# interaction-lab-uh/STROTSS-tensorflow

Measured on AMD Instinct MI355X. Metric: optimisation_steps_per_sec_1024px_pair, higher is better.
Workload: dtype f32; 1 GPU; 1024px content/style pair, 1024x1024 scale of the coarse-to-fine pyramid, 1024 samples x D=2179, VGG16 (seeded He-normal weights), RMSprop pixel update; scale_px=1024, samples=1024, parallelism=single GPU, tap_adjoint=deterministic (planned, sorted scatter)

## Files before the change

strotss-tensorflow_amd/csrc/image.hip:

```cpp
#include "internal.h"

namespace {

struct AxisTap { int lo, hi; float lerp; };
__device__ __forceinline__ AxisTap axis_tap(int i, float scale, int in_size) {
  const float src = __fsub_rn(__fmul_rn(__fadd_rn((float)i, 0.5f), scale), 0.5f);
  const float fl = floorf(src);
  AxisTap t;
  t.lo = max((int)fl, 0);
  t.hi = min((int)ceilf(src), in_size - 1);
  t.lerp = __fsub_rn(src, fl);
  return t;
}

template <int C>
__global__ __launch_bounds__(256) void resize_bilinear_kernel(const float* __restrict__ in, int ih, int iw,
                                                              int c_rt, float* __restrict__ out, int oh, int ow,
                                                              float sy, float sx, float alpha,
                                                              const float* __restrict__ add) {
  const int c = C ? C : c_rt;
  for (int oy = blockIdx.y; oy < oh; oy += gridDim.y) {
    const AxisTap ty = axis_tap(oy, sy, ih);
    const float* r0 = in + (size_t)ty.lo * iw * c;
    const float* r1 = in + (size_t)ty.hi * iw * c;
    const size_t orow = (size_t)oy * ow * c;
    for (int ox = blockIdx.x * 256 + threadIdx.x; ox < ow; ox += gridDim.x * 256) {
      const AxisTap tx = axis_tap(ox, sx, iw);
      const int a = tx.lo * c, b = tx.hi * c;
      const size_t o = orow + (size_t)ox * c;
#pragma unroll
      for (int ch = 0; ch < (C ? C : 1); ++ch)
        for (int cc = ch; cc < c; cc += (C ? C : 1)) {
          const float tl = r0[a + cc], tr = r0[b + cc], bl = r1[a + cc], br = r1[b + cc];
          const float top = tl + (tr - tl) * tx.lerp;
          const float bot = bl + (br - bl) * tx.lerp;
          float v = alpha * (top + (bot - top) * ty.lerp);
          if (add) v += add[o + cc];
          out[o + cc] = v;
        }
    }
  }
}

#define FOLD_TILE 32
#define FOLD_REGION 24
struct FoldLevels { int n; int h[STROTSS_MAX_TENSORS], w[STROTSS_MAX_TENSORS]; const float* v[STROTSS_MAX_TENSORS]; };
__device__ __forceinline__ float bilerp3(float tl, float tr, float bl, float br, float lx, float ly) {
  const float top = tl + (tr - tl) * lx;
  const float bot = bl + (br - bl) * lx;
  return 1.0f * (top + (bot - top) * ly);
}
__global__ __launch_bounds__(256) void fold_pyramid_kernel(FoldLevels p, float* __restrict__ img) {
  __shared__ float buf[2][FOLD_REGION * FOLD_REGION * 3];
  __shared__ int reg[STROTSS_MAX_TENSORS][4];
  const int t = threadIdx.x;
  if (t == 0) {
    int y0 = blockIdx.y * FOLD_TILE, y1 = min(y0 + FOLD_TILE, p.h[0]) - 1;
    int x0 = blockIdx.x * FOLD_TILE, x1 = min(x0 + FOLD_TILE, p.w[0]) - 1;
    reg[0][0] = y0; reg[0][1] = y1; reg[0][2] = x0; reg[0][3] = x1;
    for (int k = 1; k < p.n; ++k) {
      const float sy = (float)p.h[k] / (float)p.h[k - 1], sx = (float)p.w[k] / (float)p.w[k - 1];
      const int ny0 = axis_tap(y0, sy, p.h[k]).lo, ny1 = axis_tap(y1, sy, p.h[k]).hi;
      const int nx0 = axis_tap(x0, sx, p.w[k]).lo, nx1 = axis_tap(x1, sx, p.w[k]).hi;
      y0 = ny0; y1 = ny1; x0 = nx0; x1 = nx1;
      reg[k][0] = y0; reg[k][1] = y1; reg[k][2] = x0; reg[k][3] = x1;
    }
  }
  __syncthreads();
  {
    const int k = p.n - 1, y0 = reg[k][0], x0 = reg[k][2], rh = reg[k][1] - y0 + 1, rw = reg[k][3] - x0 + 1;
    float* dst = buf[k & 1];
    for (int e = t; e < rh * rw; e += 256) {
      const int ry = e / rw, rx = e - ry * rw;
      const float* s = p.v[k] + ((size_t)(y0 + ry) * p.w[k] + x0 + rx) * 3;
      dst[e * 3 + 0] = s[0]; dst[e * 3 + 1] = s[1]; dst[e * 3 + 2] = s[2];
    }
  }
  __syncthreads();
  for (int k = p.n - 2; k >= 0; --k) {
    const int y0 = reg[k][0], x0 = reg[k][2], rh = reg[k][1] - y0 + 1, rw = reg[k][3] - x0 + 1;
    const int cy0 = reg[k + 1][0], cx0 = reg[k + 1][2], cw = reg[k + 1][3] - cx0 + 1;
    const int ih = p.h[k + 1], iw = p.w[k + 1];
    const float sy = (float)ih / (float)p.h[k], sx = (float)iw / (float)p.w[k];
    const float* src = buf[(k + 1) & 1];
    float* dst = k == 0 ? nullptr : buf[k & 1];
    for (int e = t; e < rh * rw; e += 256) {
      const int ry = e / rw, rx = e - ry * rw;
      const int oy = y0 + ry, ox = x0 + rx;
      const AxisTap ty = axis_tap(oy, sy, ih), tx = axis_tap(ox, sx, iw);
      const float* r0 = src + (size_t)(ty.lo - cy0) * cw * 3;
      const float* r1 = src + (size_t)(ty.hi - cy0) * cw * 3;
      const int a = (tx.lo - cx0) * 3, b = (tx.hi - cx0) * 3;
      const size_t o = ((size_t)oy * p.w[k] + ox) * 3;
      const float* add = p.v[k] + o;
#pragma unroll
      for (int c = 0; c < 3; ++c) {
        float v = bilerp3(r0[a + c], r0[b + c], r1[a + c], r1[b + c], tx.lerp, ty.lerp);
        v += add[c];
        if (k == 0) img[o + c] = v; else dst[e * 3 + c] = v;
      }
    }
    __syncthreads();
  }
}

#define ADJ_MAX 8
__device__ __forceinline__ float adj_weight(int o, float scale, int in_size, int i) {
  const AxisTap t = axis_tap(o, scale, in_size);
  return (t.lo == i ? 1.0f - t.lerp : 0.f) + (t.hi == i ? t.lerp : 0.f);
}
struct AdjGlobal3 {
  const float* p; int ow;
  __device__ __forceinline__ const float* at(int oy, int ox) const { return p + ((size_t)oy * ow + ox) * 3; }
};
struct AdjRegion3 {
  const float* p; int y0, x0, rw;
  __device__ __forceinline__ const float* at(int oy, int ox) const { return p + ((oy - y0) * rw + (ox - x0)) * 3; }
};
__device__ __forceinline__ void adj_range(int i, float inv_scale, int out_size, int& o0, int& o1) {
  o0 = max(0, (int)floorf(((float)i - 0.5f) * inv_scale - 0.5f) - 1);
  o1 = min(out_size - 1, (int)ceilf(((float)i + 1.5f) * inv_scale - 0.5f) + 1);
}
template <class Src>
__device__ __forceinline__ void adjoint_pixel3(const Src& g, int oh, int ow, int ih, int iw, float sy, float sx, int iy,
                                               int ix, float (&acc)[3]) {
  int oy0, oy1, ox0, ox1;
  adj_range(iy, 1.0f / sy, oh, oy0, oy1);
  adj_range(ix, 1.0f / sx, ow, ox0, ox1);
  acc[0] = acc[1] = acc[2] = 0.f;
  if (ox1 - ox0 < ADJ_MAX) {
    float wx[ADJ_MAX];
#pragma unroll
    for (int q = 0; q < ADJ_MAX; ++q) wx[q] = (ox0 + q <= ox1) ? adj_weight(ox0 + q, sx, iw, ix) : 0.f;
    for (int oy = oy0; oy <= oy1; ++oy) {
      const float wy = adj_weight(oy, sy, ih, iy);
      if (wy == 0.f) continue;
      float row[3] = {0.f, 0.f, 0.f};
#pragma unroll
      for (int q = 0; q < ADJ_MAX; ++q)
        if (wx[q] != 0.f) {
          const float* p = g.at(oy, ox0 + q);
#pragma unroll
          for (int ch = 0; ch < 3; ++ch) row[ch] += wx[q] * p[ch];
        }
#pragma unroll
      for (int ch = 0; ch < 3; ++ch) acc[ch] += wy * row[ch];
    }
    return;
  }
  for (int oy = oy0; oy <= oy1; ++oy) {
    const float wy = adj_weight(oy, sy, ih, iy);
    if (wy == 0.f) continue;
    float row[3] = {0.f, 0.f, 0.f};
    for (int ox = ox0; ox <= ox1; ++ox) {
      const float w = adj_weight(ox, sx, iw, ix);
      if (w != 0.f) {
        const float* q = g.at(oy, ox);
#pragma unroll
        for (int ch = 0; ch < 3; ++ch) row[ch] += w * q[ch];
      }
    }
#pragma unroll
    for (int ch = 0; ch < 3; ++ch) acc[ch] += wy * row[ch];
  }
}

#define ADJ2_T2 8
#define ADJ2_REGION 32
__global__ __launch_bounds__(256) void resize_adjoint_pair_kernel(const float* __restrict__ g0, int h0, int w0,
                                                                  float* __restrict__ g1, int h1, int w1,
                                                                  float* __restrict__ g2, int h2, int w2) {
  __shared__ float mid[ADJ2_REGION * ADJ2_REGION * 3];
  const int t = threadIdx.x;
  const float sy1 = (float)h1 / (float)h0, sx1 = (float)w1 / (float)w0;
  const float sy2 = (float)h2 / (float)h1, sx2 = (float)w2 / (float)w1;
  const int ty0 = blockIdx.y * ADJ2_T2, ty1 = min(ty0 + ADJ2_T2, h2) - 1, tx0 = blockIdx.x * ADJ2_T2, tx1 = min(tx0 + ADJ2_T2, w2) - 1;
  const int oy0 = blockIdx.y * 2 * ADJ2_T2, oy1 = min(oy0 + 2 * ADJ2_T2, h1) - 1;
  const int ox0 = blockIdx.x * 2 * ADJ2_T2, ox1 = min(ox0 + 2 * ADJ2_T2, w1) - 1;
  const bool has2 = ty0 <= ty1 && tx0 <= tx1, own1 = oy0 <= oy1 && ox0 <= ox1;
  int ry0 = oy0, ry1 = oy1, rx0 = ox0, rx1 = ox1;
  if (has2) {
    int a, b, c, d;
    adj_range(ty0, 1.0f / sy2, h1, a, b); adj_range(ty1, 1.0f / sy2, h1, c, d);
    const int ny0 = a, ny1 = d;
    adj_range(tx0, 1.0f / sx2, w1, a, b); adj_range(tx1, 1.0f / sx2, w1, c, d);
    const int nx0 = a, nx1 = d;
    if (own1) { ry0 = min(ry0, ny0); ry1 = max(ry1, ny1); rx0 = min(rx0, nx0); rx1 = max(rx1, nx1); }
    else { ry0 = ny0; ry1 = ny1; rx0 = nx0; rx1 = nx1; }
  } else if (!own1) {
    return;
  }
  const int rh = ry1 - ry0 + 1, rw = rx1 - rx0 + 1;
  const AdjGlobal3 src0{g0, w0};
  for (int e = t; e < rh * rw; e += 256) {
    const int ry = e / rw, rx = e - ry * rw;
    const int iy = ry0 + ry, ix = rx0 + rx;
    float acc[3];
    adjoint_pixel3(src0, h0, w0, h1, w1, sy1, sx1, iy, ix, acc);
    mid[e * 3 + 0] = acc[0]; mid[e * 3 + 1] = acc[1]; mid[e * 3 + 2] = acc[2];
    if (own1 && iy >= oy0 && iy <= oy1 && ix >= ox0 && ix <= ox1) {
      float* o = g1 + ((size_t)iy * w1 + ix) * 3;
      o[0] = acc[0]; o[1] = acc[1]; o[2] = acc[2];
    }
  }
  __syncthreads();
  if (!has2) return;
  const AdjRegion3 src1{mid, ry0, rx0, rw};
  const int th = ty1 - ty0 + 1, tw = tx1 - tx0 + 1;
  for (int e = t; e < th * tw; e += 256) {
    const int iy = ty0 + e / tw, ix = tx0 + e % tw;
    float acc[3];
    adjoint_pixel3(src1, h1, w1, h2, w2, sy2, sx2, iy, ix, acc);
    float* o = g2 + ((size_t)iy * w2 + ix) * 3;
    o[0] = acc[0]; o[1] = acc[1]; o[2] = acc[2];
  }
}

template <int C>
__global__ __launch_bounds__(256) void resize_adjoint_kernel(const float* __restrict__ gout, int oh, int ow,
                                                             int c_rt, float* __restrict__ gin, int ih, int iw,
                                                             float sy, float sx) {
  const int c = C ? C : c_rt;
  const float isy = 1.0f / sy, isx = 1.0f / sx;
  for (int iy = blockIdx.y; iy < ih; iy += gridDim.y) {
    const int oy0 = max(0, (int)floorf(((float)iy - 0.5f) * isy - 0.5f) - 1);
    const int oy1 = min(oh - 1, (int)ceilf(((float)iy + 1.5f) * isy - 0.5f) + 1);
    for (int ix = blockIdx.x * 256 + threadIdx.x; ix < iw; ix += gridDim.x * 256) {
      const int ox0 = max(0, (int)floorf(((float)ix - 0.5f) * isx - 0.5f) - 1);
      const int ox1 = min(ow - 1, (int)ceilf(((float)ix + 1.5f) * isx - 0.5f) + 1);
      float acc[C ? C : 4];
#pragma unroll
      for (int ch = 0; ch < (C ? C : 4); ++ch) acc[ch] = 0.f;
      if (C && ox1 - ox0 < ADJ_MAX) {
        float wx[ADJ_MAX];
#pragma unroll
        for (int q = 0; q < ADJ_MAX; ++q) wx[q] = (ox0 + q <= ox1) ? adj_weight(ox0 + q, sx, iw, ix) : 0.f;
        for (int oy = oy0; oy <= oy1; ++oy) {
          const float wy = adj_weight(oy, sy, ih, iy);
          if (wy == 0.f) continue;
          const float* g = gout + ((size_t)oy * ow + ox0) * c;
          float row[C ? C : 1];
#pragma unroll
          for (int ch = 0; ch < C; ++ch) row[ch] = 0.f;
#pragma unroll
          for (int q = 0; q < ADJ_MAX; ++q)
            if (wx[q] != 0.f) {
#pragma unroll
              for (int ch = 0; ch < C; ++ch) row[ch] += wx[q] * g[q * c + ch];
            }
#pragma unroll
          for (int ch = 0; ch < C; ++ch) acc[ch] += wy * row[ch];
        }
#pragma unroll
        for (int ch = 0; ch < C; ++ch) gin[((size_t)iy * iw + ix) * c + ch] = acc[ch];
      } else {
        for (int ch0 = 0; ch0 < c; ch0 += 4) {
          const int nc = min(4, c - ch0);
          float a4[4] = {0.f, 0.f, 0.f, 0.f};
          for (int oy = oy0; oy <= oy1; ++oy) {
            const float wy = adj_weight(oy, sy, ih, iy);
            if (wy == 0.f) continue;
            float row[4] = {0.f, 0.f, 0.f, 0.f};
            for (int ox = ox0; ox <= ox1; ++ox) {
              const float w = adj_weight(ox, sx, iw, ix);
              if (w != 0.f)
                for (int ch = 0; ch < nc; ++ch) row[ch] += w * gout[((size_t)oy * ow + ox) * c + ch0 + ch];
            }
            for (int ch = 0; ch < nc; ++ch) a4[ch] += wy * row[ch];
          }
          for (int ch = 0; ch < nc; ++ch) gin[((size_t)iy * iw + ix) * c + ch0 + ch] = a4[ch];
        }
      }
    }
  }
}

struct SampleTap { int ia, ib, ic, id; float wa, wb, wc, wd; };

__device__ __forceinline__ SampleTap sample_tap(const strotss_maps_t& m, int k, float gx, float gy,
                                                int bilinear) {
  for (int q = 0; q < m.n_div[k]; ++q) {
    gx = __fdiv_rn(gx, m.div[q]);
    gy = __fdiv_rn(gy, m.div[q]);
  }
  const int h = m.h[k], w = m.w[k];
  SampleTap t;
  if (bilinear) {
    const float gxf = floorf(gx), gyf = floorf(gy);
    const float dx = gx - gxf, dy = gy - gyf;
    t.wa = (1.f - dx) * (1.f - dy);
    t.wb = (1.f - dx) * dy;
    t.wc = dx * (1.f - dy);
    t.wd = dx * dy;
    const int x0 = (int)fminf(fmaxf(gxf, 0.f), (float)(h - 1));
    const int y0 = (int)fminf(fmaxf(gyf, 0.f), (float)(w - 1));
    int x1 = min(x0 + 1, h - 1);
    const int y1 = min(y0 + 1, w - 1);
    int xa = x0;
    if (m.rows[k] > 0) {
      const int ra = x0 - m.row0[k], rb = x1 - m.row0[k];
      xa = min(max(ra, 0), m.rows[k] - 1);
      x1 = min(max(rb, 0), m.rows[k] - 1);
      if (m.window_drop & (int)(ra != xa)) { t.wa = 0.f; t.wb = 0.f; }
      if (m.window_drop & (int)(rb != x1)) { t.wc = 0.f; t.wd = 0.f; }
    }
    t.ia = xa * w + y0; t.ib = xa * w + y1; t.ic = x1 * w + y0; t.id = x1 * w + y1;
  } else {
    int xi = (int)fminf(fmaxf(gx, 0.f), (float)(h - 1));
    const int yi = (int)fminf(fmaxf(gy, 0.f), (float)(w - 1));
    if (m.rows[k] > 0) xi = min(max(xi - m.row0[k], 0), m.rows[k] - 1);
    t.ia = t.ib = t.ic = t.id = xi * w + yi;
    t.wa = 1.f; t.wb = t.wc = t.wd = 0.f;
  }
  return t;
}

__device__ __forceinline__ void gather_row(const strotss_maps_t& m, const float* __restrict__ idx, int s, int bilinear,
                                           float* __restrict__ out, int ld, int dtotal) {
  if (m.sample_range && (s < m.sample_range[0] || s >= m.sample_range[1])) return;
  const float gx = idx[2 * s], gy = idx[2 * s + 1];
  float* o = out + (size_t)s * ld;
  const int wave = __builtin_amdgcn_readfirstlane((int)threadIdx.x >> 6), lane = threadIdx.x & 63;
  int off = 0, chunk = 0;
  for (int k = 0; k < m.n_maps; ++k) {
    const int c = m.c[k], nchunk = (c + 63) >> 6;
    int q0 = (wave - chunk) & 3;
    if (q0 < nchunk) {
      const SampleTap t = sample_tap(m, k, gx, gy, bilinear);
      const float* src = m.map[k];
      if (bilinear) {
        const float* pa = src + (size_t)t.ia * c; const float* pb = src + (size_t)t.ib * c;
        const float* pc = src + (size_t)t.ic * c; const float* pd = src + (size_t)t.id * c;
        for (int q = q0; q < nchunk; q += 4) {
          const int ch = q * 64 + lane;
          if (ch < c) o[off + ch] = pa[ch] * t.wa + pb[ch] * t.wb + pc[ch] * t.wc + pd[ch] * t.wd;
        }
      } else {
        const float* pa = src + (size_t)t.ia * c;
        for (int q = q0; q < nchunk; q += 4) {
          const int ch = q * 64 + lane;
          if (ch < c) o[off + ch] = pa[ch];
        }
      }
    }
    off += c;
    chunk += nchunk;
  }
  for (int ch = dtotal + threadIdx.x; ch < ld; ch += 256) o[ch] = 0.f;
}
__global__ __launch_bounds__(256) void hypercol_gather_kernel(strotss_maps_t m, const float* __restrict__ idx,
                                                              int bilinear, float* __restrict__ out, int ld,
                                                              int dtotal) {
  gather_row(m, idx, blockIdx.x, bilinear, out, ld, dtotal);
}
__device__ __forceinline__ void gather2_body(const strotss_maps_t& ma, const strotss_maps_t& mb,
                                             const float* __restrict__ idx, int n, int bilinear, float* __restrict__ out_a,
                                             float* __restrict__ out_b, int ld, int dtotal_a, int dtotal_b,
                                             float* __restrict__ zero, int zero_rows, const int b) {
  if (b < n) {
    gather_row(ma, idx, b, bilinear, out_a, ld, dtotal_a);
    if (zero) {
      const int r1 = b == n - 1 ? zero_rows : min(b + 1, zero_rows);
      for (int r = b; r < r1; ++r)
        for (int ch = threadIdx.x; ch < ld; ch += 256) zero[(size_t)r * ld + ch] = 0.f;
    }
  } else {
    gather_row(mb, idx, b - n, bilinear, out_b, ld, dtotal_b);
  }
}
__global__ __launch_bounds__(256) void hypercol_gather2_kernel(strotss_maps_t ma, strotss_maps_t mb,
                                                               const float* __restrict__ idx, int n, int bilinear,
                                                               float* __restrict__ out_a, float* __restrict__ out_b, int ld,
                                                               int dtotal_a, int dtotal_b, float* __restrict__ zero,
                                                               int zero_rows) {
  gather2_body(ma, mb, idx, n, bilinear, out_a, out_b, ld, dtotal_a, dtotal_b, zero, zero_rows, (int)blockIdx.x);
}
__global__ __launch_bounds__(256) void hypercol_gather2_cw_kernel(strotss_maps_t ma, strotss_maps_t mb, strotss_maps_t mw,
                                                                  const float* __restrict__ idx, int n, int bilinear,
                                                                  float* __restrict__ out_a, float* __restrict__ out_b, int ld,
                                                                  int dtotal_a, int dtotal_b, float* __restrict__ zero,
                                                                  int zero_rows, float* __restrict__ wout, int wrows) {
  const int b = blockIdx.x;
  gather2_body(ma, mb, idx, n, bilinear, out_a, out_b, ld, dtotal_a, dtotal_b, zero, zero_rows, b);
  if (b < n) {
    gather_row(mw, idx, b, bilinear, wout, 1, 1);
    if (b == n - 1)
      for (int r = n + (int)threadIdx.x; r < wrows; r += 256) wout[r] = 0.f;
  }
}
#define SCATTER_DENSE_MAX_PIX 64
__device__ __forceinline__ void scatter_dense_block(const strotss_maps_t& m, const float* __restrict__ idx, int n,
                                                    const float* __restrict__ gfeat, int ld, bool masked, int k, int off, int b) {
  __shared__ int li[1024];
  __shared__ float lw[1024];
  __shared__ int cnts[4];
  __shared__ float red[4][64];
  const int tid = threadIdx.x, lane = tid & 63, wave = tid >> 6;
  const int c = m.c[k], nchunk = (c + 63) >> 6;
  const int p = b / nchunk, q = b - p * nchunk;
  const int s0 = m.sample_range ? m.sample_range[0] : 0, s1 = m.sample_range ? min(n, m.sample_range[1]) : n;
  const int ch = q * 64 + lane;
  const bool in = ch < c;
  const float* g = gfeat + off + (in ? ch : c - 1);
  float acc = 0.f;
  for (int base = s0; base < s1; base += 1024) {
    float w4[4];
    int cnt = 0;
#pragma unroll
    for (int u = 0; u < 4; ++u) {
      const int s = base + 4 * tid + u;
      float w = 0.f;
      if (s < s1) {
        const SampleTap t = sample_tap(m, k, idx[2 * s], idx[2 * s + 1], 1);
        w = (t.ia == p ? t.wa : 0.f) + (t.ib == p ? t.wb : 0.f) + (t.ic == p ? t.wc : 0.f) + (t.id == p ? t.wd : 0.f);
      }
      w4[u] = w;
      cnt += w != 0.f;
    }
    int incl = cnt;
#pragma unroll
    for (int o = 1; o < 64; o <<= 1) {
      const int up = __shfl_up(incl, o, 64);
      if (lane >= o) incl += up;
    }
    __syncthreads();
    if (lane == 63) cnts[wave] = incl;
    __syncthreads();
    int at = incl - cnt, total = 0;
#pragma unroll
    for (int wv = 0; wv < 4; ++wv) {
      at += wv < wave ? cnts[wv] : 0;
      total += cnts[wv];
    }
#pragma unroll
    for (int u = 0; u < 4; ++u)
      if (w4[u] != 0.f) { li[at] = base + 4 * tid + u; lw[at] = w4[u]; ++at; }
    __syncthreads();
    int e = wave;
    for (; e + 12 < total; e += 16) {
      float v[4];
#pragma unroll
      for (int u = 0; u < 4; ++u) v[u] = g[(size_t)li[e + 4 * u] * ld];
#pragma unroll
      for (int u = 0; u < 4; ++u) acc += lw[e + 4 * u] * v[u];
    }
    for (; e < total; e += 4) acc += lw[e] * g[(size_t)li[e] * ld];
  }
  red[wave][lane] = acc;
  __syncthreads();
  if (wave == 0 && in) {
    const float tot = (red[0][lane] + red[1][lane]) + (red[2][lane] + red[3][lane]);
    const size_t o = (size_t)p * c + ch;
    if (tot != 0.f && (!masked || m.map[k][o] > 0.f)) m.gmap[k][o] += tot;
  }
}
__global__ __launch_bounds__(256) void hypercol_scatter_kernel(strotss_maps_t m, const float* __restrict__ idx,
                                                               const float* __restrict__ gfeat, int ld,
                                                               int relu_mask_from, int map_begin,
                                                               int map_end, int n, unsigned dense_mask, int dense_blocks) {
  if ((int)blockIdx.x < dense_blocks) {
    int b = (int)blockIdx.x, off = 0;
    for (int k = 0; k < map_end; ++k) {
      if ((dense_mask >> k) & 1u) {
        const int nb = (m.rows[k] > 0 ? m.rows[k] : m.h[k]) * m.w[k] * ((m.c[k] + 63) >> 6);
        if (b < nb) { scatter_dense_block(m, idx, n, gfeat, ld, k >= relu_mask_from, k, off, b); return; }
        b -= nb;
      }
      off += m.c[k];
    }
    return;
  }
  const int s = (int)blockIdx.x - dense_blocks;
  if (m.sample_range && (s < m.sample_range[0] || s >= m.sample_range[1])) return;
  const float gx = idx[2 * s], gy = idx[2 * s + 1];
  const float* g = gfeat + (size_t)s * ld;
  const int wave = __builtin_amdgcn_readfirstlane((int)threadIdx.x >> 6), lane = threadIdx.x & 63;
  int off = 0, chunk = 0;
  for (int k = 0; k < map_end; ++k) {
    const int c = m.c[k], nchunk = (c + 63) >> 6;
    const int q0 = (wave - chunk) & 3;
    chunk += nchunk;
    if (k < map_begin || q0 >= nchunk || ((dense_mask >> k) & 1u)) { off += c; continue; }
    const SampleTap t = sample_tap(m, k, gx, gy, 1);
    const float* act = m.map[k];
    float* dst = m.gmap[k];
    const bool masked = k >= relu_mask_from;
    const int ii[4] = {t.ia, t.ib, t.ic, t.id};
    const float ww[4] = {t.wa, t.wb, t.wc, t.wd};
    for (int q = q0; q < nchunk; q += 4) {
      const int ch = q * 64 + lane;
      const bool in = ch < c;
      const int chc = in ? ch : c - 1;
      const float gv = in ? g[off + chc] : 0.f;
#pragma unroll
      for (int tq = 0; tq < 4; ++tq) {
        const float v = ww[tq] * gv;
        const size_t o = (size_t)ii[tq] * c + chc;
        if (v != 0.f && (!masked || act[o] > 0.f)) atomicAdd(&dst[o], v);
      }
    }
    off += c;
  }
}

#define PLAN_E 4096
struct PlanView {
  int* nseg; int* seg_start; int* pix; int* smp; float* w;
  __host__ __device__ static size_t ints_per_map() { return 2 + (PLAN_E + 1) + 3 * (size_t)PLAN_E + 1; }
  __host__ __device__ PlanView(void* base, int k) {
    int* b = reinterpret_cast<int*>(base) + (size_t)k * ints_per_map();
    nseg = b; seg_start = b + 2; pix = seg_start + PLAN_E + 1; smp = pix + PLAN_E; w = reinterpret_cast<float*>(smp + PLAN_E);
  }
};
__global__ __launch_bounds__(1024) void scatter_plan_kernel(strotss_maps_t m, const float* __restrict__ idx, int n,
                                                            void* __restrict__ plan) {
  __shared__ unsigned long long key[PLAN_E];
  __shared__ int wsum[16];
  const int k = blockIdx.x, t = threadIdx.x;
  const unsigned long long INVALID = ~0ull;
  const int s_begin = m.sample_range ? m.sample_range[0] : 0, s_end = m.sample_range ? min(n, m.sample_range[1]) : n;
  for (int e = t; e < PLAN_E; e += 1024) {
    const int s = e >> 2, q = e & 3;
    unsigned long long kk = INVALID;
    if (s >= s_begin && s < s_end) {
      const SampleTap tp = sample_tap(m, k, idx[2 * s], idx[2 * s + 1], 1);
      const int ii = q == 0 ? tp.ia : q == 1 ? tp.ib : q == 2 ? tp.ic : tp.id;
      const float ww = q == 0 ? tp.wa : q == 1 ? tp.wb : q == 2 ? tp.wc : tp.wd;
      if (ww != 0.f) kk = ((unsigned long long)(unsigned)ii << 12) | (unsigned)e;
    }
    key[e] = kk;
  }
  __syncthreads();
  for (int size = 2; size <= PLAN_E; size <<= 1)
    for (int stride = size >> 1; stride > 0; stride >>= 1) {
      for (int p = t; p < PLAN_E / 2; p += 1024) {
        const int lo = 2 * p - (p & (stride - 1));
        const int hi = lo + stride;
        const bool up = (lo & size) == 0;
        const unsigned long long a = key[lo], b = key[hi];
        if ((a > b) == up) { key[lo] = b; key[hi] = a; }
      }
      __syncthreads();
    }
  PlanView pv(plan, k);
  int head[4], cnt = 0, valid = 0;
#pragma unroll
  for (int i = 0; i < 4; ++i) {
    const int p = 4 * t + i;
    const unsigned long long a = key[p];
    const bool ok = a != INVALID;
    head[i] = ok && (p == 0 || (key[p - 1] >> 12) != (a >> 12));
    cnt += head[i]; valid += ok;
  }
  int incl = cnt, vincl = valid;
#pragma unroll
  for (int o = 1; o < 64; o <<= 1) {
    const int u = __shfl_up(incl, o, 64), v = __shfl_up(vincl, o, 64);
    if ((t & 63) >= o) { incl += u; vincl += v; }
  }
  if ((t & 63) == 63) { wsum[t >> 6] = incl; }
  __syncthreads();
  int base = incl - cnt;
  for (int wv = 0; wv < (t >> 6); ++wv) base += wsum[wv];
  int total = 0;
#pragma unroll
  for (int wv = 0; wv < 16; ++wv) total += wsum[wv];
  __syncthreads();
  if ((t & 63) == 63) wsum[t >> 6] = vincl;
  __syncthreads();
  int nvalid = 0;
#pragma unroll
  for (int wv = 0; wv < 16; ++wv) nvalid += wsum[wv];
#pragma unroll
  for (int i = 0; i < 4; ++i) {
    const int p = 4 * t + i;
    const unsigned long long a = key[p];
    if (a == INVALID) continue;
    const int e = (int)(a & 4095u), s = e >> 2, q = e & 3;
    const SampleTap tp = sample_tap(m, k, idx[2 * s], idx[2 * s + 1], 1);
    pv.pix[p] = (int)(a >> 12);
    pv.smp[p] = s;
    pv.w[p] = q == 0 ? tp.wa : q == 1 ? tp.wb : q == 2 ? tp.wc : tp.wd;
    if (head[i]) pv.seg_start[base++] = p;
  }
  if (t == 0) { pv.nseg[0] = total; pv.seg_start[total] = nvalid; }
}
__global__ __launch_bounds__(256) void scatter_sorted_kernel(strotss_maps_t m, int k, int off, const void* __restrict__ plan,
                                                             const float* __restrict__ gfeat, int ld, int masked) {
  PlanView pv(const_cast<void*>(plan), k);
  const int sg = blockIdx.x;
  if (sg >= pv.nseg[0]) return;
  const int p0 = pv.seg_start[sg], p1 = pv.seg_start[sg + 1];
  const int c = m.c[k];
  const size_t pixel = (size_t)pv.pix[p0] * c;
  const float* act = m.map[k];
  float* dst = m.gmap[k];
  for (int ch = threadIdx.x; ch < c; ch += 256) {
    if (masked && !(act[pixel + ch] > 0.f)) continue;
    float acc = 0.f;
    for (int p = p0; p < p1; ++p) acc += pv.w[p] * gfeat[(size_t)pv.smp[p] * ld + off + ch];
    dst[pixel + ch] += acc;
  }
}

__global__ __launch_bounds__(256) void rmsprop_kernel(strotss_tensors_t t, float lr, float rho, float eps) {
  const int k = blockIdx.y;
  float* var = t.var[k];
  float* rms = t.rms[k];
  const float* g = t.grad[k];
  const int64_t n = t.numel[k];
  const float omr = 1.0f - rho;
  for (int64_t e = (int64_t)blockIdx.x * 256 + threadIdx.x; e < n; e += (int64_t)gridDim.x * 256) {
    const float gv = g[e];
    const float r = rho * rms[e] + omr * (gv * gv);
    rms[e] = r;
    var[e] = var[e] - lr * gv / (sqrtf(r) + eps);
  }
}

__global__ __launch_bounds__(256) void minmax_partial_kernel(const float* __restrict__ x, int64_t n,
                                                             float* __restrict__ ws) {
  __shared__ float red[4];
  float mn = INFINITY, mx = -INFINITY;
  for (int64_t e = (int64_t)blockIdx.x * 256 + threadIdx.x; e < n; e += (int64_t)gridDim.x * 256) {
    const float v = fminf(fmaxf(x[e], 0.f), 1.f);
    mn = fminf(mn, v);
    mx = fmaxf(mx, v);
  }
  mn = block_min_256(mn, red);
  mx = block_max_256(mx, red);
  if (threadIdx.x == 0) { ws[blockIdx.x] = mn; ws[1024 + blockIdx.x] = mx; }
}
__global__ __launch_bounds__(256) void postprocess_kernel(const float* __restrict__ x, int64_t n,
                                                          const float* __restrict__ ws, int nparts,
                                                          uint8_t* __restrict__ out) {
  __shared__ float red[4];
  float mn = INFINITY, mx = -INFINITY;
  for (int i = threadIdx.x; i < nparts; i += 256) { mn = fminf(mn, ws[i]); mx = fmaxf(mx, ws[1024 + i]); }
  mn = block_min_256(mn, red);
  mx = block_max_256(mx, red);
  const float range = mx - mn;
  for (int64_t e = (int64_t)blockIdx.x * 256 + threadIdx.x; e < n; e += (int64_t)gridDim.x * 256) {
    float v = fminf(fmaxf(x[e], 0.f), 1.f);
    v = (v - mn) / range;
    out[e] = (uint8_t)(v * 255.0f);
  }
}

int maps_ok(const strotss_maps_t* m) {
  if (!m || m->n_maps <= 0 || m->n_maps > STROTSS_MAX_MAPS) return 0;
  for (int k = 0; k < m->n_maps; ++k) {
    if (m->h[k] <= 0 || m->w[k] <= 0 || m->c[k] <= 0 || !m->map[k]) return 0;
    if (m->n_div[k] < 0 || m->n_div[k] > STROTSS_MAX_DIVS) return 0;
    if (m->rows[k] < 0 || m->row0[k] < 0 || m->row0[k] + m->rows[k] > m->h[k]) return 0;
  }
  return 1;
}

}

extern "C" {

int strotss_abi_version(void) { return 8; }
const char* strotss_build_info(void) { return "libstrotss_hip gfx950 fp32-mfma " __DATE__ " " __TIME__; }

int strotss_resize_bilinear(const float* in, int ih, int iw, int c, float* out, int oh, int ow, float alpha,
                            const float* add, void* stream) {
  ST_CHECK_ARG(in && out && ih > 0 && iw > 0 && oh > 0 && ow > 0 && c > 0, STROTSS_EINVAL);
  const float sy = (float)ih / (float)oh, sx = (float)iw / (float)ow;
  const dim3 grid((unsigned)cdiv(ow, 256), (unsigned)min(oh, 32768));
  if (c == 3)
    hipLaunchKernelGGL(resize_bilinear_kernel<3>, grid, dim3(256), 0, (hipStream_t)stream, in, ih, iw, c, out, oh, ow, sy, sx,
                       alpha, add);
  else if (c == 1)
    hipLaunchKernelGGL(resize_bilinear_kernel<1>, grid, dim3(256), 0, (hipStream_t)stream, in, ih, iw, c, out, oh, ow, sy, sx,
                       alpha, add);
  else
    hipLaunchKernelGGL(resize_bilinear_kernel<0>, grid, dim3(256), 0, (hipStream_t)stream, in, ih, iw, c, out, oh, ow, sy, sx,
                       alpha, add);
  ST_LAUNCH_RET();
}

int strotss_fold_pyramid(const strotss_pyramid_t* pyr, float* img, void* stream) {
  ST_CHECK_ARG(pyr && img && pyr->n_levels >= 2 && pyr->n_levels <= STROTSS_MAX_TENSORS, STROTSS_EINVAL);
  FoldLevels p;
  p.n = pyr->n_levels;
  for (int k = 0; k < p.n; ++k) {
    ST_CHECK_ARG(pyr->var[k] && pyr->h[k] > 0 && pyr->w[k] > 0, STROTSS_EINVAL);
    p.h[k] = pyr->h[k]; p.w[k] = pyr->w[k]; p.v[k] = pyr->var[k];
  }
  int sy = FOLD_TILE, sx = FOLD_TILE;
  for (int k = 1; k < p.n; ++k) {
    ST_CHECK_ARG(p.h[k] <= p.h[k - 1] && p.w[k] <= p.w[k - 1], STROTSS_ERANGE);
    sy = min(p.h[k], (int)((long long)sy * p.h[k] / p.h[k - 1]) + 3);
    sx = min(p.w[k], (int)((long long)sx * p.w[k] / p.w[k - 1]) + 3);
    ST_CHECK_ARG(sy <= FOLD_REGION && sx <= FOLD_REGION, STROTSS_ERANGE);
  }
  hipLaunchKernelGGL(fold_pyramid_kernel, dim3((unsigned)cdiv(p.w[0], FOLD_TILE), (unsigned)cdiv(p.h[0], FOLD_TILE)), dim3(256),
                     0, (hipStream_t)stream, p, img);
  ST_LAUNCH_RET();
}

static bool adjoint_pair_ok(int a, int b) { return b >= 1 && a >= 2 * b - 1 && a <= 2 * b + 1; }

int strotss_fold_pyramid_adjoint(const strotss_pyramid_t* g, void* stream) {
  ST_CHECK_ARG(g && g->n_levels >= 2 && g->n_levels <= STROTSS_MAX_TENSORS, STROTSS_EINVAL);
  for (int k = 0; k < g->n_levels; ++k) ST_CHECK_ARG(g->var[k] && g->h[k] > 0 && g->w[k] > 0, STROTSS_EINVAL);
  int k = 0;
  while (k + 1 < g->n_levels) {
    const bool pair = k + 2 < g->n_levels && adjoint_pair_ok(g->h[k], g->h[k + 1]) && adjoint_pair_ok(g->w[k], g->w[k + 1]) &&
                      adjoint_pair_ok(g->h[k + 1], g->h[k + 2]) && adjoint_pair_ok(g->w[k + 1], g->w[k + 2]);
    if (pair) {
      const unsigned gx = (unsigned)max(cdiv(g->w[k + 2], ADJ2_T2), cdiv(g->w[k + 1], 2 * ADJ2_T2));
      const unsigned gy = (unsigned)max(cdiv(g->h[k + 2], ADJ2_T2), cdiv(g->h[k + 1], 2 * ADJ2_T2));
      hipLaunchKernelGGL(resize_adjoint_pair_kernel, dim3(gx, gy), dim3(256), 0, (hipStream_t)stream,
                         (const float*)g->var[k], g->h[k], g->w[k], const_cast<float*>(g->var[k + 1]), g->h[k + 1], g->w[k + 1],
                         const_cast<float*>(g->var[k + 2]), g->h[k + 2], g->w[k + 2]);
      k += 2;
    } else {
      const int rc = strotss_resize_bilinear_adjoint(g->var[k], g->h[k], g->w[k], 3, const_cast<float*>(g->var[k + 1]),
                                                     g->h[k + 1], g->w[k + 1], stream);
      if (rc != 0) return rc;
      k += 1;
    }
  }
  ST_LAUNCH_RET();
}

int strotss_resize_bilinear_adjoint(const float* gout, int oh, int ow, int c, float* gin, int ih, int iw,
                                    void* stream) {
  ST_CHECK_ARG(gout && gin && ih > 0 && iw > 0 && oh > 0 && ow > 0 && c > 0, STROTSS_EINVAL);
  const float sy = (float)ih / (float)oh, sx = (float)iw / (float)ow;
  const dim3 grid((unsigned)cdiv(iw, 256), (unsigned)min(ih, 32768));
  if (c == 3)
    hipLaunchKernelGGL(resize_adjoint_kernel<3>, grid, dim3(256), 0, (hipStream_t)stream, gout, oh, ow, c, gin, ih, iw, sy, sx);
  else if (c == 1)
    hipLaunchKernelGGL(resize_adjoint_kernel<1>, grid, dim3(256), 0, (hipStream_t)stream, gout, oh, ow, c, gin, ih, iw, sy, sx);
  else
    hipLaunchKernelGGL(resize_adjoint_kernel<0>, grid, dim3(256), 0, (hipStream_t)stream, gout, oh, ow, c, gin, ih, iw, sy, sx);
  ST_LAUNCH_RET();
}

int strotss_hypercol_gather(const strotss_maps_t* maps, const float* idx, int n, int bilinear, float* out,
                            int ld, void* stream) {
  ST_CHECK_ARG(maps_ok(maps) && idx && out && n > 0, STROTSS_EINVAL);
  int d = 0;
  for (int k = 0; k < maps->n_maps; ++k) d += maps->c[k];
  ST_CHECK_ARG(ld >= d, STROTSS_EINVAL);
  strotss_maps_t m = *maps;
  m.window_drop = 0;
  hipLaunchKernelGGL(hypercol_gather_kernel, dim3(n), dim3(256), 0, (hipStream_t)stream, m, idx, bilinear,
                     out, ld, d);
  ST_LAUNCH_RET();
}

int strotss_hypercol_gather2(const strotss_maps_t* maps_a, const strotss_maps_t* maps_b, const float* idx, int n,
                             int bilinear, float* out_a, float* out_b, int ld, float* zero, int zero_rows, void* stream) {
  ST_CHECK_ARG(maps_ok(maps_a) && maps_ok(maps_b) && idx && out_a && out_b && n > 0, STROTSS_EINVAL);
  ST_CHECK_ARG(!zero || zero_rows > 0, STROTSS_EINVAL);
  int da = 0, db = 0;
  for (int k = 0; k < maps_a->n_maps; ++k) da += maps_a->c[k];
  for (int k = 0; k < maps_b->n_maps; ++k) db += maps_b->c[k];
  ST_CHECK_ARG(ld >= da && ld >= db, STROTSS_EINVAL);
  strotss_maps_t a = *maps_a, b = *maps_b;
  a.window_drop = b.window_drop = 0;
  hipLaunchKernelGGL(hypercol_gather2_kernel, dim3(2 * n), dim3(256), 0, (hipStream_t)stream, a, b, idx, n, bilinear, out_a,
                     out_b, ld, da, db, zero, zero_rows);
  ST_LAUNCH_RET();
}

int strotss_hypercol_gather2_cw(const strotss_maps_t* maps_a, const strotss_maps_t* maps_b, const strotss_maps_t* maps_w,
                                const float* idx, int n, int bilinear, float* out_a, float* out_b, int ld, float* zero,
                                int zero_rows, float* weight_out, int weight_rows, void* stream) {
  ST_CHECK_ARG(maps_ok(maps_a) && maps_ok(maps_b) && maps_ok(maps_w) && idx && out_a && out_b && weight_out && n > 0,
               STROTSS_EINVAL);
  ST_CHECK_ARG(maps_w->n_maps == 1 && maps_w->c[0] == 1 && maps_w->rows[0] == 0 && weight_rows >= n, STROTSS_EINVAL);
  ST_CHECK_ARG(!zero || zero_rows > 0, STROTSS_EINVAL);
  int da = 0, db = 0;
  for (int k = 0; k < maps_a->n_maps; ++k) da += maps_a->c[k];
  for (int k = 0; k < maps_b->n_maps; ++k) db += maps_b->c[k];
  ST_CHECK_ARG(ld >= da && ld >= db, STROTSS_EINVAL);
  strotss_maps_t a = *maps_a, b = *maps_b, wm = *maps_w;
  a.window_drop = b.window_drop = wm.window_drop = 0;
  wm.sample_range = nullptr;
  hipLaunchKernelGGL(hypercol_gather2_cw_kernel, dim3(2 * n), dim3(256), 0, (hipStream_t)stream, a, b, wm, idx, n, bilinear,
                     out_a, out_b, ld, da, db, zero, zero_rows, weight_out, weight_rows);
  ST_LAUNCH_RET();
}

int strotss_hypercol_scatter(const strotss_maps_t* maps, const float* idx, int n, const float* gfeat, int ld,
                             int relu_mask_from, int map_begin, int map_end, void* stream) {
  ST_CHECK_ARG(maps_ok(maps) && idx && gfeat && n > 0, STROTSS_EINVAL);
  ST_CHECK_ARG(map_begin >= 0 && map_begin < map_end && map_end <= maps->n_maps, STROTSS_ERANGE);
  int d = 0;
  for (int k = 0; k < maps->n_maps; ++k) {
    if (k >= map_begin && k < map_end) ST_CHECK_ARG(maps->gmap[k] != nullptr, STROTSS_EINVAL);
    d += maps->c[k];
  }
  ST_CHECK_ARG(ld >= d, STROTSS_EINVAL);
  static const int dense_pix = [] {
    const char* e = getenv("STROTSS_SCATTER_DENSE");
    const int v = e ? atoi(e) : 1;
    return v == 1 ? SCATTER_DENSE_MAX_PIX : v;
  }();
  unsigned dense_mask = 0;
  int dense_blocks = 0;
  for (int k = map_begin; k < map_end; ++k) {
    const int pix = (maps->rows[k] > 0 ? maps->rows[k] : maps->h[k]) * maps->w[k];
    if (pix <= dense_pix) { dense_mask |= 1u << k; dense_blocks += pix * ((maps->c[k] + 63) / 64); }
  }
  hipLaunchKernelGGL(hypercol_scatter_kernel, dim3(n + dense_blocks), dim3(256), 0, (hipStream_t)stream, *maps, idx, gfeat,
                     ld, relu_mask_from, map_begin, map_end, n, dense_mask, dense_blocks);
  ST_LAUNCH_RET();
}

size_t strotss_hypercol_scatter_plan_bytes(int n_maps) {
  return n_maps > 0 ? (size_t)n_maps * PlanView::ints_per_map() * sizeof(int) : 0;
}

int strotss_hypercol_scatter_plan(const strotss_maps_t* maps, const float* idx, int n, void* plan, size_t plan_bytes,
                                  void* stream) {
  ST_CHECK_ARG(maps_ok(maps) && idx && plan && n > 0, STROTSS_EINVAL);
  ST_CHECK_ARG(4 * n <= PLAN_E, STROTSS_ERANGE);
  ST_CHECK_ARG(plan_bytes >= strotss_hypercol_scatter_plan_bytes(maps->n_maps), STROTSS_EINVAL);
  for (int k = 0; k < maps->n_maps; ++k) {
    const long long px = (long long)(maps->rows[k] > 0 ? maps->rows[k] : maps->h[k]) * maps->w[k];
    ST_CHECK_ARG(px < (1ll << 31), STROTSS_ERANGE);
  }
  hipLaunchKernelGGL(scatter_plan_kernel, dim3(maps->n_maps), dim3(1024), 0, (hipStream_t)stream, *maps, idx, n, plan);
  ST_LAUNCH_RET();
}

int strotss_hypercol_scatter_sorted(const strotss_maps_t* maps, const void* plan, int n, const float* gfeat, int ld,
                                    int relu_mask_from, int map_begin, int map_end, void* stream) {
  ST_CHECK_ARG(maps_ok(maps) && plan && gfeat && n > 0 && 4 * n <= PLAN_E, STROTSS_EINVAL);
  ST_CHECK_ARG(map_begin >= 0 && map_begin < map_end && map_end <= maps->n_maps, STROTSS_ERANGE);
  int off = 0;
  for (int k = 0; k < map_end; ++k) {
    if (k >= map_begin) {
      ST_CHECK_ARG(maps->gmap[k] != nullptr && off + maps->c[k] <= ld, STROTSS_EINVAL);
      hipLaunchKernelGGL(scatter_sorted_kernel, dim3(4 * n), dim3(256), 0, (hipStream_t)stream, *maps, k, off, plan, gfeat,
                         ld, k >= relu_mask_from ? 1 : 0);
    }
    off += maps->c[k];
  }
  ST_LAUNCH_RET();
}

int strotss_rmsprop_step(const strotss_tensors_t* t, float lr, float rho, float eps, void* stream) {
  ST_CHECK_ARG(t && t->n_tensors > 0 && t->n_tensors <= STROTSS_MAX_TENSORS, STROTSS_ERANGE);
  int64_t mx = 0;
  for (int k = 0; k < t->n_tensors; ++k) {
    ST_CHECK_ARG(t->var[k] && t->rms[k] && t->grad[k] && t->numel[k] > 0, STROTSS_EINVAL);
    mx = t->numel[k] > mx ? t->numel[k] : mx;
  }
  dim3 grid((unsigned)((mx + 255) / 256 > 2048 ? 2048 : (mx + 255) / 256), t->n_tensors);
  hipLaunchKernelGGL(rmsprop_kernel, grid, dim3(256), 0, (hipStream_t)stream, *t, lr, rho, eps);
  ST_LAUNCH_RET();
}

int strotss_postprocess(const float* img, int64_t numel, uint8_t* out, float* workspace, void* stream) {
  ST_CHECK_ARG(img && out && workspace && numel > 0, STROTSS_EINVAL);
  const int nparts = (int)((numel + 255) / 256 > 1024 ? 1024 : (numel + 255) / 256);
  hipLaunchKernelGGL(minmax_partial_kernel, dim3(nparts), dim3(256), 0, (hipStream_t)stream, img, numel,
                     workspace);
  hipLaunchKernelGGL(postprocess_kernel, dim3(nparts), dim3(256), 0, (hipStream_t)stream, img, numel,
                     workspace, nparts, out);
  ST_LAUNCH_RET();
}

}
```

strotss-tensorflow_amd/csrc/sort_match.h:

```cpp
#pragma once
#include "common.h"

namespace {

constexpr int SORT_T = 1024;

__device__ __forceinline__ unsigned long long ordered_pack(float v, int idx) {
  unsigned b = __float_as_uint(v);
  if (b == 0x80000000u) b = 0u;
  const unsigned key = (b & 0x80000000u) ? ~b : (b | 0x80000000u);
  return ((unsigned long long)key << 32) | (unsigned)idx;
}
__device__ __forceinline__ float ordered_value(unsigned long long c) {
  const unsigned key = (unsigned)(c >> 32);
  return __uint_as_float((key & 0x80000000u) ? (key & 0x7FFFFFFFu) : ~key);
}

template <int SIDES>
__device__ __forceinline__ void bitonic_sort_1024(unsigned long long (&v)[SIDES], unsigned long long* buf0,
                                                  unsigned long long* buf1, int S) {
  const int tid = threadIdx.x;
  int cross = 0;
#pragma unroll
  for (int k = 2; k <= SORT_T; k <<= 1) {
#pragma unroll
    for (int j = k >> 1; j > 0; j >>= 1) {
      unsigned long long* const buf = (cross & 1) ? buf1 : buf0;
      if (j >= 64) ++cross;
      if (k > S) continue;
      unsigned long long pv[SIDES];
      if (j < 64) {
#pragma unroll
        for (int s = 0; s < SIDES; ++s)
          pv[s] = ((unsigned long long)__shfl_xor((unsigned)(v[s] >> 32), j, 64) << 32) | __shfl_xor((unsigned)v[s], j, 64);
      } else {
#pragma unroll
        for (int s = 0; s < SIDES; ++s) buf[s * SORT_T + tid] = v[s];
        __syncthreads();
#pragma unroll
        for (int s = 0; s < SIDES; ++s) pv[s] = buf[s * SORT_T + (tid ^ j)];
      }
      const bool keep_low = ((tid & j) == 0) == ((tid & k) == 0);
#pragma unroll
      for (int s = 0; s < SIDES; ++s) v[s] = (v[s] < pv[s]) == keep_low ? v[s] : pv[s];
    }
  }
}

struct SquaredCost {
  static __device__ __forceinline__ void pair(float len, float diff, float& g, float& w) {
    g += len * diff;
    w += len * diff * diff;
  }
};
struct AbsoluteCost {
  static __device__ __forceinline__ void pair(float len, float diff, float& g, float& w) {
    g += diff > 0.f ? len : (diff < 0.f ? -len : 0.f);
    w += len * fabsf(diff);
  }
};

struct QuantileMatch {
  float coef;
  int row;
  float cost;
};

template <class Cost>
__device__ __forceinline__ QuantileMatch quantile_match(unsigned long long va, unsigned long long vb, int n, int ns,
                                                        float* sb) {
  const int tid = threadIdx.x;
  if (tid < ns) sb[tid] = ordered_value(vb);
  __syncthreads();
  QuantileMatch m = {0.f, 0, 0.f};
  if (tid < n) {
    const float a = ordered_value(va);
    const int lo = tid * ns, hi = lo + ns;
    float g = 0.f, w = 0.f;
    for (int j = lo / n; j < ns && j * n < hi; ++j) {
      const float len = (float)(min(hi, (j + 1) * n) - max(lo, j * n));
      const float diff = a - sb[j];
      Cost::pair(len, diff, g, w);
    }
    const float inv = (float)(1.0 / ((double)n * ns));
    m.coef = g * inv;
    m.row = (int)(unsigned)(va & 0xFFFFFFFFull);
    m.cost = w * inv;
  }
  return m;
}

__device__ __forceinline__ double block_sum_f64_1024(double v, double* red) {
  const int tid = threadIdx.x;
  v = wave_sum(v);
  if ((tid & 63) == 0) red[tid >> 6] = v;
  __syncthreads();
  double s = 0.0;
  if (tid == 0) {
#pragma unroll
    for (int i = 0; i < SORT_T / 64; ++i) s += red[i];
  }
  return s;
}

}
```

Measured before the change: 231.7 steps/s.

## Sort scatter-plan keys in registers with wave shuffles instead of shared-memory bitonic passes

The scatter-plan kernel now holds four keys per thread in registers and sorts them with a register/shuffle bitonic network. Only strides of 64 threads or more go through double-buffered shared memory, which removes most of the per-stage block barriers and LDS round trips of the old shared-array bitonic sort. The tap weights are cached in shared memory, so the final write no longer recomputes sample_tap per element. The prefix-sum barriers are also merged. The cost is more shared memory (two 4096-entry buffers plus a weight array), and this kernel is a small part of each optimisation step.

```diff
diff --git a/strotss-tensorflow_amd/csrc/image.hip b/strotss-tensorflow_amd/csrc/image.hip
--- a/strotss-tensorflow_amd/csrc/image.hip
+++ b/strotss-tensorflow_amd/csrc/image.hip
@@ -1,4 +1,5 @@
 #include "internal.h"
+#include "sort_match.h"
 
 namespace {
 
@@ -514,73 +515,62 @@
 };
 __global__ __launch_bounds__(1024) void scatter_plan_kernel(strotss_maps_t m, const float* __restrict__ idx, int n,
                                                             void* __restrict__ plan) {
-  __shared__ unsigned long long key[PLAN_E];
-  __shared__ int wsum[16];
-  const int k = blockIdx.x, t = threadIdx.x;
+  __shared__ unsigned long long buf0[PLAN_E], buf1[PLAN_E];
+  __shared__ float wl[PLAN_E];
+  __shared__ unsigned edge[16];
+  __shared__ int wsum[2][16];
+  const int k = blockIdx.x, t = threadIdx.x, lane = t & 63, wave = t >> 6;
   const unsigned long long INVALID = ~0ull;
   const int s_begin = m.sample_range ? m.sample_range[0] : 0, s_end = m.sample_range ? min(n, m.sample_range[1]) : n;
-  for (int e = t; e < PLAN_E; e += 1024) {
-    const int s = e >> 2, q = e & 3;
-    unsigned long long kk = INVALID;
-    if (s >= s_begin && s < s_end) {
-      const SampleTap tp = sample_tap(m, k, idx[2 * s], idx[2 * s + 1], 1);
-      const int ii = q == 0 ? tp.ia : q == 1 ? tp.ib : q == 2 ? tp.ic : tp.id;
-      const float ww = q == 0 ? tp.wa : q == 1 ? tp.wb : q == 2 ? tp.wc : tp.wd;
-      if (ww != 0.f) kk = ((unsigned long long)(unsigned)ii << 12) | (unsigned)e;
-    }
-    key[e] = kk;
-  }
+  unsigned long long v[4] = {INVALID, INVALID, INVALID, INVALID};
+  if (t >= s_begin && t < s_end) {
+    const SampleTap tp = sample_tap(m, k, idx[2 * t], idx[2 * t + 1], 1);
+    const int ii[4] = {tp.ia, tp.ib, tp.ic, tp.id};
+    const float ww[4] = {tp.wa, tp.wb, tp.wc, tp.wd};
+#pragma unroll
+    for (int q = 0; q < 4; ++q) {
+      if (ww[q] != 0.f) v[q] = ((unsigned long long)(unsigned)ii[q] << 12) | (unsigned)(4 * t + q);
+      wl[4 * t + q] = ww[q];
+    }
+  }
+  bitonic_sort_4096(v, buf0, buf1);
+  unsigned prev = __shfl_up((unsigned)(v[3] >> 12), 1, 64);
+  if (lane == 63) edge[wave] = (unsigned)(v[3] >> 12);
   __syncthreads();
-  for (int size = 2; size <= PLAN_E; size <<= 1)
-    for (int stride = size >> 1; stride > 0; stride >>= 1) {
-      for (int p = t; p < PLAN_E / 2; p += 1024) {
-        const int lo = 2 * p - (p & (stride - 1));
-        const int hi = lo + stride;
-        const bool up = (lo & size) == 0;
-        const unsigned long long a = key[lo], b = key[hi];
-        if ((a > b) == up) { key[lo] = b; key[hi] = a; }
-      }
-      __syncthreads();
-    }
+  if (lane == 0 && wave > 0) prev = edge[wave - 1];
+  int head[4], cnt = 0, valid = 0;
+#pragma unroll
+  for (int i = 0; i < 4; ++i) {
+    const unsigned px = (unsigned)(v[i] >> 12);
+    const bool ok = v[i] != INVALID;
+    head[i] = ok && ((t == 0 && i == 0) || prev != px);
+    cnt += head[i]; valid += ok;
+    prev = px;
+  }
+  int incl = cnt, vincl = valid;
+#pragma unroll
+  for (int o = 1; o < 64; o <<= 1) {
+    const int u = __shfl_up(incl, o, 64), w = __shfl_up(vincl, o, 64);
+    if (lane >= o) { incl += u; vincl += w; }
+  }
+  if (lane == 63) { wsum[0][wave] = incl; wsum[1][wave] = vincl; }
+  __syncthreads();
+  int base = incl - cnt, total = 0, nvalid = 0;
+#pragma unroll
+  for (int wv = 0; wv < 16; ++wv) {
+    base += wv < wave ? wsum[0][wv] : 0;
+    total += wsum[0][wv];
+    nvalid += wsum[1][wv];
+  }
   PlanView pv(plan, k);
-  int head[4], cnt = 0, valid = 0;
 #pragma unroll
   for (int i = 0; i < 4; ++i) {
     const int p = 4 * t + i;
-    const unsigned long long a = key[p];
-    const bool ok = a != INVALID;
-    head[i] = ok && (p == 0 || (key[p - 1] >> 12) != (a >> 12));
-    cnt += head[i]; valid += ok;
-  }
-  int incl = cnt, vincl = valid;
-#pragma unroll
-  for (int o = 1; o < 64; o <<= 1) {
-    const int u = __shfl_up(incl, o, 64), v = __shfl_up(vincl, o, 64);
-    if ((t & 63) >= o) { incl += u; vincl += v; }
-  }
-  if ((t & 63) == 63) { wsum[t >> 6] = incl; }
-  __syncthreads();
-  int base = incl - cnt;
-  for (int wv = 0; wv < (t >> 6); ++wv) base += wsum[wv];
-  int total = 0;
-#pragma unroll
-  for (int wv = 0; wv < 16; ++wv) total += wsum[wv];
-  __syncthreads();
-  if ((t & 63) == 63) wsum[t >> 6] = vincl;
-  __syncthreads();
-  int nvalid = 0;
-#pragma unroll
-  for (int wv = 0; wv < 16; ++wv) nvalid += wsum[wv];
-#pragma unroll
-  for (int i = 0; i < 4; ++i) {
-    const int p = 4 * t + i;
-    const unsigned long long a = key[p];
-    if (a == INVALID) continue;
-    const int e = (int)(a & 4095u), s = e >> 2, q = e & 3;
-    const SampleTap tp = sample_tap(m, k, idx[2 * s], idx[2 * s + 1], 1);
-    pv.pix[p] = (int)(a >> 12);
-    pv.smp[p] = s;
-    pv.w[p] = q == 0 ? tp.wa : q == 1 ? tp.wb : q == 2 ? tp.wc : tp.wd;
+    if (v[i] == INVALID) continue;
+    const int e = (int)(v[i] & 4095u);
+    pv.pix[p] = (int)(v[i] >> 12);
+    pv.smp[p] = e >> 2;
+    pv.w[p] = wl[e];
     if (head[i]) pv.seg_start[base++] = p;
   }
   if (t == 0) { pv.nseg[0] = total; pv.seg_start[total] = nvalid; }
diff --git a/strotss-tensorflow_amd/csrc/sort_match.h b/strotss-tensorflow_amd/csrc/sort_match.h
--- a/strotss-tensorflow_amd/csrc/sort_match.h
+++ b/strotss-tensorflow_amd/csrc/sort_match.h
@@ -43,6 +43,51 @@
       const bool keep_low = ((tid & j) == 0) == ((tid & k) == 0);
 #pragma unroll
       for (int s = 0; s < SIDES; ++s) v[s] = (v[s] < pv[s]) == keep_low ? v[s] : pv[s];
+    }
+  }
+}
+
+__device__ __forceinline__ void sort_pair(unsigned long long& a, unsigned long long& b, bool up) {
+  const unsigned long long lo = a < b ? a : b, hi = a < b ? b : a;
+  a = up ? lo : hi;
+  b = up ? hi : lo;
+}
+
+__device__ __forceinline__ void bitonic_sort_4096(unsigned long long (&v)[4], unsigned long long* buf0,
+                                                  unsigned long long* buf1) {
+  const int tid = threadIdx.x;
+  int cross = 0;
+#pragma unroll
+  for (int k = 2; k <= 4 * SORT_T; k <<= 1) {
+    const bool up = ((4 * tid) & k) == 0;
+#pragma unroll
+    for (int j = k >> 1; j > 0; j >>= 1) {
+      if (j == 1) {
+        sort_pair(v[0], v[1], up);
+        sort_pair(v[2], v[3], k == 2 ? false : up);
+      } else if (j == 2) {
+        sort_pair(v[0], v[2], up);
+        sort_pair(v[1], v[3], up);
+      } else {
+        const int m = j >> 2;
+        unsigned long long pv[4];
+        if (m < 64) {
+#pragma unroll
+          for (int i = 0; i < 4; ++i)
+            pv[i] = ((unsigned long long)__shfl_xor((unsigned)(v[i] >> 32), m, 64) << 32) | __shfl_xor((unsigned)v[i], m, 64);
+        } else {
+          unsigned long long* const buf = (cross & 1) ? buf1 : buf0;
+          ++cross;
+#pragma unroll
+          for (int i = 0; i < 4; ++i) buf[i * SORT_T + tid] = v[i];
+          __syncthreads();
+#pragma unroll
+          for (int i = 0; i < 4; ++i) pv[i] = buf[i * SORT_T + (tid ^ m)];
+        }
+        const bool keep_low = ((tid & m) == 0) == up;
+#pragma unroll
+        for (int i = 0; i < 4; ++i) v[i] = (v[i] < pv[i]) == keep_low ? v[i] : pv[i];
+      }
     }
   }
 }
```

New measurement: 232.5 steps/s (median of 6 runs). About the same (+0.4%).
